# SpursLipu/YOLOv3v4-ModelCompression-MultidatasetTraining-Multibackbone

Hardware: AMD Instinct MI355X
Metric: images/sec YOLOv3-608 train fp16 (higher is better)
Workload: dtype f16; 1 GPU; YOLOv3 Darknet-53 608 COCO (80 classes) fp16 training step, batch 64/GPU: train-mode forward (batch-stat BN) + compute_loss + backward + nesterov SGD, single GPU; global_batch=64, parallelism=dp1

## Files before the change

yolov3v4-modelcompression-multidatasettraining-multibackbone_amd/csrc/conv_halo_pp.hip:

```cpp
#include "conv_igemm.h"

namespace yh {

template <typename T> struct HppMma;
template <> struct HppMma<f16> {
    typedef f16x8 frag_t;
    static __device__ __forceinline__ f32x4 mma(const frag_t& a, const frag_t& b, const f32x4& c) {
        return __builtin_amdgcn_mfma_f32_16x16x32_f16(a, b, c, 0, 0, 0);
    }
};
template <> struct HppMma<int8_t> {
    typedef i32x4 frag_t;
    static __device__ __forceinline__ i32x4 mma(const frag_t& a, const frag_t& b, const i32x4& c) {
        return __builtin_amdgcn_mfma_i32_16x16x64_i8(a, b, c, 0, 0, 0);
    }
};

template <typename T, int ACT, typename AccT>
__device__ __forceinline__ void hpp_epilogue(const ConvArgs& a, AccT (&acc)[8][4], const f32x4 (&bvs)[8], const long (&pix)[4],
                                             const int m0, const long tile_row, const int lane, float* const stage) {
    constexpr int TM = 8, TN = 4;
    const int mq = (lane >> 4) << 2, pc = lane & 15;
    T* const yg = reinterpret_cast<T*>(a.y);
    const T* const rg = reinterpret_cast<const T*>(a.res);
    const int mbase = m0 + mq;
    auto value = [&](auto ic, auto jc, int e) {
        constexpr int i = decltype(ic)::value, j = decltype(jc)::value;
        if constexpr (sizeof(T) == 1) {
            const float y = activate_q<ACT>((float)acc[i][j][e] * a.acc_scale + bvs[i][e], a.slope, a.inv_out_scale);
            return round_clamp_i8(y * a.inv_out_scale);
        } else {
            return activate_t<ACT, T>((float)acc[i][j][e] + bvs[i][e], a.slope);
        }
    };
    if constexpr (sizeof(T) != 1) {
        if (a.stats_part != nullptr) {
// ... 6 lines not shown
                    if (pix[j] >= 0) {
#pragma unroll
                        for (int e = 0; e < 4; ++e) {
                            const float q = (float)(T)value(ic, jc, e);
                            s1[e] += q;
                            s2[e] = fmaf(q, q, s2[e]);
                        }
                    }
                });
#pragma unroll
                for (int e = 0; e < 4; ++e) {
                    const float t1 = row16_sum(s1[e]), t2 = row16_sum(s2[e]);
                    const int m = mbase + i * 16 + e;
                    if (pc == 15 && stage != nullptr) {
                        stage[i * 16 + mq + e] = t1;
                        stage[128 + i * 16 + mq + e] = t2;
                    } else if (pc == 15 && m < a.Cout) {
                        row[m] = t1;
                        row[a.Cout + m] = t2;
                    }
                }
            });
            __builtin_amdgcn_wave_barrier();
            if (stage != nullptr) {
                const int half = lane >> 5, c4 = (lane & 31) * 4;
                const f32x4 sv = *reinterpret_cast<const f32x4*>(stage + half * 128 + c4);
                if (m0 + c4 < a.Cout) *reinterpret_cast<f32x4*>(row + half * a.Cout + m0 + c4) = sv;
            }
        }
    }
    const int k4 = lane >> 4;
    const int chan = ((k4 & 1) << 4) + ((k4 >> 1) << 3);
    const bool have_res = rg != nullptr;
    static_for<TN>([&](auto jc) {
        constexpr int j = decltype(jc)::value;
        const long p = pix[j];
        typedef unsigned int u32x2 __attribute__((ext_vector_type(2)));
        typedef typename std::conditional<sizeof(T) == 2, u32x4, u32x2>::type res8_t;
        res8_t rv[TM / 2];
        if (have_res) {
#pragma unroll
            for (int i2 = 0; i2 < TM / 2; ++i2) {
// ... 51 lines not shown
                }
                u32x2 o;
#pragma unroll
                for (int h = 0; h < 2; ++h)
                    o[h] = ((unsigned)(int)v[4 * h] & 0xffu) | (((unsigned)(int)v[4 * h + 1] & 0xffu) << 8) |
                           (((unsigned)(int)v[4 * h + 2] & 0xffu) << 16) | (((unsigned)(int)v[4 * h + 3] & 0xffu) << 24);
                *reinterpret_cast<u32x2*>(prow + m) = o;
            }
        });
    });
}

template <int T9, int LB> struct HppAllow {
    static constexpr int in(int t) { return (t >= 0 && t < LB) ? 1 : 0; }
    static constexpr int value = T9 == 8 ? 2 : 2 + in(T9 - 2) + in(T9 - 1) + in(T9);
};

template <int T9, int LB> struct HppAllow2 {
    static constexpr int in(int t) { return (t >= 0 && t < LB) ? 1 : 0; }
    static constexpr int end = T9 >= 7 ? 1 : 1 + in(T9 - 1) + in(T9);
    static constexpr int mid = T9 >= 7 ? 1 : 1 + in(T9 - 1);
};

struct HppDiv { unsigned m_img, s_img, m_wp, s_wp; };
__device__ __forceinline__ int hpp_div(int n, unsigned m, unsigned s) { return (int)(__umulhi((unsigned)n, m) >> s); }

template <typename T, int LB, int ROLE, int KFORM>
__global__ __launch_bounds__(512, 2) void conv3x3_hpp_kernel(const ConvArgs a, const int rows_hp, const int hbufs_arg, const HppDiv dv) {
    const int hbufs = hbufs_arg & 0xff;
    constexpr bool ONEBAR = KFORM == 1, REFRESH = KFORM == 2;
    constexpr int VEC = Prec<T>::VEC, BK = VEC * 4;
    constexpr int BM = 128, BN = 512, TM = 8, TN = 4, NW = 8, SA = 4;
    constexpr int A_CELLS = BM * 4;
    constexpr int LBR = ROLE ? 1 : LB;
    static_assert(sizeof(T) <= 2, "f16 / int8");
    typedef typename HppMma<T>::frag_t frag_t;
    typedef typename AccOf<T>::type acc_t;
    typedef const void __attribute__((address_space(1))) * gptr_t;
    typedef void __attribute__((address_space(3))) * lptr_t;

    extern __shared__ __attribute__((aligned(16))) u32x4 hsm[];
    u32x4* const Aring = hsm;
    u32x4* const Hbuf = hsm + SA * A_CELLS;
    u32x4* const dummy = Hbuf + hbufs * rows_hp * 4;
    int* const htab = reinterpret_cast<int*>(dummy + 64);

    const int lane = threadIdx.x & 63;
    const int wave = __builtin_amdgcn_readfirstlane(threadIdx.x >> 6);
    const int group = wave >> 2;

// ... 6 lines not shown
    {
        const int nb = gridDim.x, bid = blockIdx.x;
        const int q = nb >> 3, rr = nb & 7, xcd = bid & 7;
        const int logical = (xcd < rr ? xcd * (q + 1) : rr * (q + 1) + (xcd - rr) * q) + (bid >> 3);
        p_tile = logical / a.m_tiles;
        m_tile = logical - p_tile * a.m_tiles;
    }
    const int m0 = m_tile * BM;
    const long q0 = (long)p_tile * BN;
    const int Wp = a.W + 1;
    const int IMG = (a.H + 1) * Wp;

    const int lrow = lane >> 2;
    const int lu = (lane & 3) ^ (((lane >> 4) & 1) << 1);
    const T* const xg = reinterpret_cast<const T*>(a.x);
    const int wrow = (ROLE ? 2 * (wave & 3) : wave) * 16 + lrow;
    const T* const wsrc = reinterpret_cast<const T*>(a.w) + (long)min(m0 + wrow, a.m_pad - 1) * a.ktot + lu * VEC;
    const int wsrc2 = (min(m0 + wrow + 16, a.m_pad - 1) - min(m0 + wrow, a.m_pad - 1)) * a.ktot;
    auto halo_offset = [&](int j) {
        const int v = (int)q0 - Wp - 1 + j;
        int off = -1;
        if (j < rows_hp && v >= 0) {
            const int n = hpp_div(v, dv.m_img, dv.s_img);
            const int rem = v - n * IMG;
            const int yy = hpp_div(rem, dv.m_wp, dv.s_wp), xx = rem - yy * Wp;
            if (n < a.N && yy >= 1 && xx >= 1) off = ((n * a.H + yy - 1) * a.W + xx - 1) * a.ldx;
        }
        return off;
    };
    int boff[LBR];
    if constexpr (ROLE == 0) {
// ... 89 lines not shown
        LOADS;                                                \
        __builtin_amdgcn_sched_barrier(0);                    \
        asm volatile("s_waitcnt lgkmcnt(0)" ::: "memory");   \
        if (BAR_L) __builtin_amdgcn_s_barrier();              \
        __builtin_amdgcn_sched_barrier(0);                    \
        MMA;                                                  \
        __builtin_amdgcn_sched_barrier(0);                    \
        if (BAR_M) __builtin_amdgcn_s_barrier();              \
        __builtin_amdgcn_sched_barrier(0);                    \
    } while (0)

    const int nchunks = a.cin_k / BK;
    const int nk = 9 * nchunks;
    if constexpr (ROLE == 0) {
        static_for<LB>([&](auto ic) { issue_h(0, 0, ic); });
        issue_a(0, 0, 0);
        issue_a(1, 1, 0);
        issue_a(2, 2, 0);
        wait_vmcnt<2>();
    } else if (group == 0) {
        issue_a(0, 0, 0);
        issue_a(1, 1, 0);
        issue_a(2, 2, 0);
        wait_vmcnt<4>();
    } else {
        for (int i = 0; i < 6; ++i) issue_h2(0, 0, i);
        wait_vmcnt<0>();
    }
    if constexpr (REFRESH) {
        static_assert(!REFRESH || ROLE == 0, "the refresh form shares the LDS-DMA issue among all waves");
        wait_vmcnt<1>();
        YH_HPP_BARRIER();
        read_a(Aring, 0);
        read_b(Hbuf, 0);
// ... 47 lines not shown
                    fb[j] = *reinterpret_cast<frag_t*>(&v);
                    __builtin_amdgcn_sched_barrier(0);
                }
                if (group == 0) {
                    if (more_h) wait_vmcnt<HppAllow2<t, LB>::end>();
                    else if (s + 3 < nk) wait_vmcnt<1>();
                    else wait_vmcnt<0>();
                    YH_HPP_BARRIER();
                }
                ++s;
                st_r = (st_r + 1) & (SA - 1);
                st_w = (st_w + 1) & (SA - 1);
                if (++ptap == 9) { ptap = 0; pkc += BK; }
            });
        }
    } else {
    YH_HPP_BARRIER();
    if (!ONEBAR && group == 1) YH_HPP_BARRIER();
    int s = 0;
    int st_r = 0, st_w = 3;
    int ptap = 3, pkc = 0;
    for (int c = 0; c < nchunks; ++c) {
        const bool more_h = LB <= 7 ? c + 1 < nchunks : false;
        const u32x4* const hb = Hbuf + (c & (hbufs - 1)) * (rows_hp * 4);
        const int nbuf = (c + 1) & 1, nkc = (c + 1) * BK;
        static_for<9>([&](auto tc) {
            constexpr int t = decltype(tc)::value;
            const u32x4* const st = Aring + st_r * A_CELLS;
            const int tapoff = (t / 3) * Wp + (t % 3);
            constexpr int allow = HppAllow<t, LB>::value;
// ... 33 lines not shown
        const int m = m0 + i * 16 + mq;
        bvs[i] = m < a.Cout ? *reinterpret_cast<const f32x4*>(a.bias + m) : f32x4{0.f, 0.f, 0.f, 0.f};
    }
#pragma unroll
    for (int i = 0; i < TM; ++i) asm volatile("" ::"v"(bvs[i]));
    long pix[TN];
#pragma unroll
    for (int j = 0; j < TN; ++j) {
        const int q = (int)q0 + wave * 64 + j * 16 + r16;
        const int n = hpp_div(q, dv.m_img, dv.s_img);
        const int rem = q - n * IMG;
        const int yy = hpp_div(rem, dv.m_wp, dv.s_wp), xx = rem - yy * Wp;
        pix[j] = (n < a.N && yy >= 1 && xx >= 1) ? ((long)n * a.H + yy - 1) * a.W + xx - 1 : -1;
    }
    const long tile_row = (long)p_tile * NW + wave;
    float* const stage = (hbufs_arg >> 8) ? reinterpret_cast<float*>(reinterpret_cast<unsigned char*>(htab) + ((rows_hp * 4 + 15) & ~15)) + wave * 256 : nullptr;
    switch (a.act) {
        case YH_ACT_LEAKY: hpp_epilogue<T, YH_ACT_LEAKY>(a, acc, bvs, pix, m0, tile_row, lane, stage); break;
        case YH_ACT_MISH: hpp_epilogue<T, YH_ACT_MISH>(a, acc, bvs, pix, m0, tile_row, lane, stage); break;
        default: hpp_epilogue<T, YH_ACT_LINEAR>(a, acc, bvs, pix, m0, tile_row, lane, stage); break;
    }
}

#ifdef YH_HPP_PERSIST_AB
template <typename T, int LB>
__global__ __launch_bounds__(512, 2) void conv3x3_hpp_persist_kernel(const ConvArgs a, const int rows_hp, const HppDiv dv, const int total_tiles) {
    constexpr int VEC = Prec<T>::VEC, BK = VEC * 4;
    constexpr int BM = 128, BN = 512, TM = 8, TN = 4, NW = 8, SA = 4;
    constexpr int A_CELLS = BM * 4;
    static_assert(sizeof(T) <= 2, "f16 / int8");
    typedef typename HppMma<T>::frag_t frag_t;
    typedef typename AccOf<T>::type acc_t;
    typedef const void __attribute__((address_space(1))) * gptr_t;
    typedef void __attribute__((address_space(3))) * lptr_t;

// ... 184 lines not shown
            bvs[i] = m < ae.Cout ? *reinterpret_cast<const f32x4*>(ae.bias + m) : f32x4{0.f, 0.f, 0.f, 0.f};
        }
#pragma unroll
        for (int i = 0; i < TM; ++i) asm volatile("" ::"v"(bvs[i]));
        long pix[TN];
#pragma unroll
        for (int j = 0; j < TN; ++j) {
            const int q = q0 + wave * 64 + j * 16 + r16;
            const int n = hpp_div(q, dv.m_img, dv.s_img);
            const int rem = q - n * IMG;
            const int yy = hpp_div(rem, dv.m_wp, dv.s_wp), xx = rem - yy * Wp;
            pix[j] = (n < a.N && yy >= 1 && xx >= 1) ? ((long)n * a.H + yy - 1) * a.W + xx - 1 : -1;
        }
        const long tile_row = (long)p_tile * NW + wave;
        switch (ae.act) {
            case YH_ACT_LEAKY: hpp_epilogue<T, YH_ACT_LEAKY>(ae, acc, bvs, pix, m0, tile_row, lane, nullptr); break;
            case YH_ACT_MISH: hpp_epilogue<T, YH_ACT_MISH>(ae, acc, bvs, pix, m0, tile_row, lane, nullptr); break;
            default: hpp_epilogue<T, YH_ACT_LINEAR>(ae, acc, bvs, pix, m0, tile_row, lane, nullptr); break;
        }
        if (!has_next) break;
        vb = vnext;
        m_tile = m_next;
        p_tile = p_next;
        wsrc = weight_off(m_next * BM);
    }
#undef YH_HPP_PHASE
#undef YH_HPP_BARRIER
}

#endif

static void hpp_magic(unsigned d, unsigned* m, unsigned* s) {
    unsigned L = 0;
    while ((1ull << L) < d) ++L;
    const unsigned long long num = 1ull << (31 + L);
    *m = (unsigned)((num + d - 1) / d);
    *s = L - 1;
}

bool hpp_geometry(int W, int cin_k, int bk, int* rows_hp, int* lb, int* hbufs, size_t* lds) {
    const int Wp = W + 1;
    const int rows_h = 512 + 2 * Wp + 2;
    *rows_hp = ((rows_h + 15) / 16) * 16;
    const int groups = *rows_hp / 16;
    int l = (groups + 7) / 8;
    const int nchunks = cin_k / bk;
    *hbufs = nchunks > 1 ? 2 : 1;
    if (l == 8) l = 9;
    if (l < 5 || l > 9 || (nchunks > 1 && l > 7)) return false;
    *lb = l;
    *lds = ((size_t)4 * 128 * 4 + (size_t)*hbufs * *rows_hp * 4 + 64) * 16 + (size_t)*rows_hp * 4;
    return *lds <= 160 * 1024;
}

template <typename T, int LBV> static auto hpp_kern(int kform) -> void (*)(const ConvArgs, const int, const int, const HppDiv) {
#ifdef YH_HPP_ONEBAR_AB
    if constexpr (!(sizeof(T) == 1 && LBV == 7)) {
        if (kform == 1) return conv3x3_hpp_kernel<T, LBV, 0, 1>;
    }
#endif
#ifdef YH_HPP_REFRESH_AB
    if constexpr (LBV <= 7) {
        if (kform == 2) return conv3x3_hpp_kernel<T, LBV, 0, 2>;
    }
#endif
    (void)kform;
    return conv3x3_hpp_kernel<T, LBV, 0, 0>;
}

#ifndef YH_HPP_ONE_BARRIER_DEFAULT
#define YH_HPP_ONE_BARRIER_DEFAULT 0
#endif
#ifndef YH_HPP_KFORM_DEFAULT
#define YH_HPP_KFORM_DEFAULT 0
#endif
template <typename T> static int launch_hpp(const ConvArgs& a0, hipStream_t stream) {
    constexpr int BK = Prec<T>::VEC * 4;
    ConvArgs a = a0;
    if (a.R != 3 || a.S != 3 || a.stride != 1 || a.pad != 1 || a.ups != 1) return YH_EUNSUPPORTED;
    if (a.act != YH_ACT_LINEAR && a.act != YH_ACT_LEAKY && a.act != YH_ACT_MISH) return YH_EUNSUPPORTED;
    if (a.cin_k % BK) return YH_EALIGN;
    int rows_hp, lb, hbufs;
    size_t lds;
    if (!hpp_geometry(a.W, a.cin_k, BK, &rows_hp, &lb, &hbufs, &lds)) return YH_EUNSUPPORTED;
    if ((long)a.N * a.H * a.W * a.ldx + a.cin_k >= 0x7fffffffL || (long)a.m_pad * a.ktot >= 0x7fffffffL) return YH_EUNSUPPORTED;
    if ((long)(a.N + 1) * (a.H + 1) * (a.W + 1) + 4096 >= 0x7fffffffL) return YH_EUNSUPPORTED;
    const unsigned amask = sizeof(T) == 2 ? 15u : 7u;
    if (a.Cout % 8 || a.ldy % 8 || (((uintptr_t)a.y) & amask) || (a.res && (a.ldr % 8 || (((uintptr_t)a.res) & amask)))) return YH_EALIGN;
    a.m_tiles = (a.Cout + 127) / 128;
    const long Q = (long)a.N * (a.H + 1) * (a.W + 1);
    a.p_tiles = (int)((Q + 511) / 512);
    const long blocks = (long)a.m_tiles * a.p_tiles;
    if (blocks <= 0 || blocks > 0x7fffffffL) return YH_EINVAL;
    int stage_ok = 0;
    if (a.stats_part != nullptr && sizeof(T) == 2) {
        const char* e = getenv("YH_HPP_STATS_STAGE");
        const size_t base = (lds + 15) & ~(size_t)15;
        if (!(e && atoi(e) == 0) && base + 8192 <= 160 * 1024) {
            lds = base + 8192;
            stage_ok = 1;
        }
    }
    { const char* e = getenv("YH_HPP_STAGGER"); a.hpp_stagger = (e && blocks > 512) ? atoi(e) : 0; }
    HppDiv dv;
    hpp_magic((unsigned)((a.H + 1) * (a.W + 1)), &dv.m_img, &dv.s_img);
    hpp_magic((unsigned)(a.W + 1), &dv.m_wp, &dv.s_wp);
    const char* bar_env = getenv("YH_HPP_BARRIERS");
    const int one_bar = bar_env ? (atoi(bar_env) == 1 ? 1 : 0) : YH_HPP_ONE_BARRIER_DEFAULT;
    const char* form_env = getenv("YH_HPP_KFORM");
    const int kform = one_bar ? 1 : (form_env ? atoi(form_env) : YH_HPP_KFORM_DEFAULT);
#ifdef YH_HPP_ROLE_AB
    static const int role_env = [] { const char* e = getenv("YH_HPP_ROLE"); return e ? atoi(e) : 0; }();
    const int role = (role_env && rows_hp <= 768) ? 1 : 0;
#define YH_HPP_KERN(LBV) (role ? conv3x3_hpp_kernel<T, LBV, 1, 0> : hpp_kern<T, LBV>(kform))
#else
#define YH_HPP_KERN(LBV) hpp_kern<T, LBV>(kform)
#endif
#define YH_HPP_CASE(LBV)                                                                                                       \
    case LBV: {                                                                                                                \
        auto kern = YH_HPP_KERN(LBV);                                                                                          \
        hipError_t e = ensure_dynamic_lds(reinterpret_cast<const void*>(kern), lds);                         \
        if (e != hipSuccess) return (int)e;                                                                                    \
        hipLaunchKernelGGL(kern, dim3((unsigned)blocks), dim3(512), lds, stream, a, rows_hp, hbufs | (stage_ok << 8), dv);     \
        break;                                                                                                                 \
    }
    switch (lb) {
        YH_HPP_CASE(5) YH_HPP_CASE(6) YH_HPP_CASE(7) YH_HPP_CASE(9)
        default: return YH_EUNSUPPORTED;
    }
#undef YH_HPP_CASE
#undef YH_HPP_KERN
// ... 35 lines not shown
    switch (lb) {
        YH_HPPP_CASE(5) YH_HPPP_CASE(6) YH_HPPP_CASE(7)
        default: return YH_EUNSUPPORTED;
    }
#undef YH_HPPP_CASE
    return check_launch();
}

int launch_hpp_persist_tile(const ConvArgs& a, int dtype, hipStream_t stream) {
    if (dtype == YH_F16) return launch_hpp_persist<f16>(a, stream);
    if (dtype == YH_I8) return launch_hpp_persist<int8_t>(a, stream);
    return YH_EINVAL;
}
#endif

int launch_hpp_tile(const ConvArgs& a, int dtype, hipStream_t stream) {
#ifdef YH_HPP_PERSIST_AB
    static const bool persist = [] { const char* e = getenv("YH_HPP_PERSIST"); return e && atoi(e) != 0; }();
    if (persist && a.R == 3 && a.S == 3 && a.stride == 1 && a.pad == 1 && a.ups == 1) {
        const int bk = dtype == YH_I8 ? 64 : 32;
        const long tiles = (long)((a.Cout + 127) / 128) * (((long)a.N * (a.H + 1) * (a.W + 1) + 511) / 512);
        if (a.cin_k % bk == 0 && a.cin_k / bk >= 2 && tiles > 256) {
            const int rc = launch_hpp_persist_tile(a, dtype, stream);
            if (rc != YH_EUNSUPPORTED) return rc;
        }
    }
#endif
    if (dtype == YH_F16) return launch_hpp<f16>(a, stream);
    if (dtype == YH_I8) return launch_hpp<int8_t>(a, stream);
    return YH_EINVAL;
}

}
```

yolov3v4-modelcompression-multidatasettraining-multibackbone_amd/csrc/conv_igemm.h:

```cpp
#pragma once
#include <type_traits>

#include "common.h"

namespace yh {

struct ConvArgs {
    const void* x;
    const void* w;
    const float* bias;
    const void* res;
    void* y;
    int N, H, W, Cin, Ho, Wo, Cout, R, S, stride, pad;
    int ldx, ldr, ldy;
    int cin_k;
    int ktot;
    long P;
    int m_tiles, p_tiles;
    int m_pad;
    float acc_scale, out_scale, inv_out_scale;
    int act;
    float slope;
    int ups;
    float* stats_part;
// ... 448 lines not shown
                    store4<OutT>(dst + (long)(c.wo2 + 1) * a.ldy, v[0], v[1], v[2], v[3]);
                }
            }
        });
    });
}

int launch_k64_tile(const ConvArgs& a, int tile, int dtype, int out_f32, hipStream_t stream);
int launch_pointwise_tile(const ConvArgs& a, int dtype, int out_f32, hipStream_t stream);
int launch_stream3_tile(const ConvArgs& a, int dtype, hipStream_t stream);
long stream3_stats_rows(long P, int cout);
int launch_pwl_tile(const ConvArgs& a, int dtype, hipStream_t stream);
bool pwl_supported(int dtype, int out_f32, int cin, int cin_k, int cout, long P, int ldx, int ldy, int ldr, const void* x, const void* y,
                   const void* res, bool stats, bool bwd);
long pwl_stats_rows(long P, int cout, bool bwd = false);
int launch_hpp_tile(const ConvArgs& a, int dtype, hipStream_t stream);
bool hpp_geometry(int W, int cin_k, int bk, int* rows_hp, int* lb, int* hbufs, size_t* lds);

}
```

yolov3v4-modelcompression-multidatasettraining-multibackbone_amd/csrc/conv_igemm.hip:

```cpp
#include "conv_igemm.h"

namespace yh {

template <typename T, int TM, int TN, int KU> struct MmaStep;

template <int TM, int TN, int KU> struct MmaStep<f16, TM, TN, KU> {
    static __device__ __forceinline__ void run(const u32x4* As, const u32x4* Bs, int BM, int BN, int arow, int brow,
                                               int lane, f32x4 (&acc)[TM][TN]) {
        const int r = lane & 15;
#pragma unroll
        for (int h = 0; h < KU / 4; ++h) {
            const int u = h * 4 + (lane >> 4);
            f16x8 a[TM], b[TN];
#pragma unroll
            for (int i = 0; i < TM; ++i) {
                u32x4 v = As[u * BM + arow + i * 16 + r];
                a[i] = *reinterpret_cast<f16x8*>(&v);
            }
#pragma unroll
            for (int j = 0; j < TN; ++j) {
                u32x4 v = Bs[u * BN + brow + j * 16 + r];
                b[j] = *reinterpret_cast<f16x8*>(&v);
            }
#pragma unroll
// ... 727 lines not shown
        case 15: return launch<T, OutT, 128, 64, 2, 2, 8>(a, s);
        case 16: return launch<T, OutT, 256, 128, 4, 2, 8>(a, s);
        case 21: return launch_glds<T, OutT, 128, 128, 2, 2, 3>(a, s);
        case 22: return launch_glds<T, OutT, 64, 256, 1, 4, 3>(a, s);
        case 24: return launch_glds<T, OutT, 64, 128, 2, 2, 3>(a, s);
        case 25: return launch_glds<T, OutT, 128, 64, 2, 2, 3>(a, s);
        case 26: return launch_glds<T, OutT, 256, 128, 4, 2, 3>(a, s);
        case 27: return launch_glds<T, OutT, 128, 256, 2, 4, 3>(a, s);
        case 51: return launch_glds<T, OutT, 256, 128, 4, 2, 3, 1>(a, s);
        case 52: return launch_glds<T, OutT, 256, 128, 4, 2, 3, 2>(a, s);
        case 41: return launch_halo<T, OutT, 128>(a, s);
        case 42: return launch_halo<T, OutT, 256>(a, s);
        case 43:
            if constexpr (sizeof(T) == 2 && std::is_same<OutT, T>::value) return launch_hpp_tile(a, YH_F16, s);
            else return YH_EUNSUPPORTED;
        case 31: return launch_glds<T, OutT, 128, 128, 2, 2, 4>(a, s);
        case 61: case 62: case 63: case 64: case 65: case 66: case 67: case 68: case 69:
            if constexpr (sizeof(T) == 2) return launch_k64_tile(a, tile, YH_F16, std::is_same<OutT, float>::value ? 1 : 0, s);
            else return YH_EINVAL;
        case 32: return launch_glds<T, OutT, 64, 256, 1, 4, 4>(a, s);
        case 34: return launch_glds<T, OutT, 64, 128, 2, 2, 4>(a, s);
        case 35: return launch_glds<T, OutT, 128, 64, 2, 2, 4>(a, s);
        default: return YH_EINVAL;
    }
}

template <typename OutT> static int dispatch_tile_i8(const ConvArgs& a, int tile, hipStream_t s) {
    if (tile == 0) {
        tile = pick_tile(a.Cout, a.P, a.cin_k, 16);
        if (tile == 3) tile = 24;
    }
    switch (tile) {
        case 21: return launch_glds<int8_t, OutT, 128, 128, 2, 2, 3>(a, s);
        case 24: return launch_glds<int8_t, OutT, 64, 128, 2, 2, 3>(a, s);
        case 25: return launch_glds<int8_t, OutT, 128, 64, 2, 2, 3>(a, s);
        case 26: return launch_glds<int8_t, OutT, 256, 128, 4, 2, 3>(a, s);
        case 27: return launch_glds<int8_t, OutT, 128, 256, 2, 4, 3>(a, s);
        case 64: case 65: case 66: return launch_k64_tile(a, tile, YH_I8, std::is_same<OutT, float>::value ? 1 : 0, s);
        case 43:
            if constexpr (std::is_same<OutT, int8_t>::value) return launch_hpp_tile(a, YH_I8, s);
            else return YH_EUNSUPPORTED;
        default: return YH_EINVAL;
    }
}

__global__ void pack_qconv_weights_kernel(const float* __restrict__ qw, float inv_scale, const int32_t* __restrict__ cin_map,
                                          int cout, int cin, int taps, int cin_k, int8_t* __restrict__ packed) {
    const long total = (long)cout * cin * taps;
    for (long i = blockIdx.x * (long)blockDim.x + threadIdx.x; i < total; i += (long)gridDim.x * blockDim.x) {
        const int tap = (int)(i % taps);
        const long r = i / taps;
        const int ci = (int)(r % cin), co = (int)(r / cin);
        const int pc = cin_map ? cin_map[ci] : ci;
        packed[((long)co * taps + tap) * cin_k + pc] = (int8_t)(int)round_clamp_i8(qw[i] * inv_scale);
    }
}
// ... 31 lines not shown
        const long blocks = (long)((d->cout + bm - 1) / bm) * ((P + bn - 1) / bn);
        return (double)((blocks + 255) / 256) * (20000.0 + 3300.0 * nk);
    };
    const double c64 = pp(256, 256), c66 = d->cout >= 512 ? pp(512, 128) : 1e30;
    const double best = c64 < c66 ? c64 : c66;
    if (best > 0.95 * ring) return 0;
    return c66 <= c64 ? 66 : 64;
}

static bool pick_halo_tile(const yh_conv_desc* d) {
    if (d->dtype != YH_F16 || d->kh != 3 || d->kw != 3 || d->stride != 1 || d->pad != 1 || d->stats_ws || d->ups > 2) return false;
    if (d->cout != 128 && d->cout != 256) return false;
    return d->cin >= 128 && d->cin % 32 == 0 && d->w_in >= 48 && d->w_in <= 96 && (long)d->n * d->h * d->w_in >= 131072;
}

static bool pick_hpp_tile(const yh_conv_desc* d) {
    static const bool off = getenv("YH_NO_HPP") != nullptr;
    if (off || (d->dtype != YH_F16 && d->dtype != YH_I8) || d->out_f32) return false;
    if (d->kh != 3 || d->kw != 3 || d->stride != 1 || d->pad != 1 || d->ups != 1) return false;
    if (d->act != YH_ACT_LINEAR && d->act != YH_ACT_LEAKY && d->act != YH_ACT_MISH) return false;
    const int bk = d->dtype == YH_I8 ? 64 : 32;
    if (d->cin_k % bk || d->cout < 64 || d->cin_k / bk < 2) return false;
    if (d->dtype == YH_F16 && d->cout <= 64 && d->cin_k / bk == 2) return false;
    if (d->dtype == YH_I8 && d->cin_k / bk == 2 && (d->res || (long)d->n * d->ho * d->wo < 262144)) return false;
    const unsigned amask = d->dtype == YH_F16 ? 15u : 7u;
    if (d->cout % 8 || d->ldy % 8 || (((uintptr_t)d->y) & amask) || (d->res && (d->ldr % 8 || (((uintptr_t)d->res) & amask)))) return false;
    if ((long)(d->n + 1) * (d->h + 1) * (d->w_in + 1) + 4096 >= 0x7fffffffL) return false;
    int rows_hp, lb, hbufs;
    size_t lds;
    if (!yh::hpp_geometry(d->w_in, d->cin_k, bk, &rows_hp, &lb, &hbufs, &lds)) return false;
    if ((long)d->n * d->h * d->w_in * d->ldx + d->cin_k >= 0x7fffffffL || (long)d->m_pad * 9 * d->cin_k >= 0x7fffffffL) return false;
    const long blocks = (long)((d->cout + 127) / 128) * (((long)d->n * (d->h + 1) * (d->w_in + 1) + 511) / 512);
    const long rounds = (blocks + 255) / 256;
    return blocks >= 192 && (rounds >= 4 || blocks * 100 >= rounds * 256 * 60);
}

static bool pick_pointwise_tile(const yh_conv_desc* d) {
    static const bool off = getenv("YH_NO_POINTWISE") != nullptr;
    if (off || (d->dtype != YH_F16 && d->dtype != YH_I8)) return false;
    if (d->kh != 1 || d->kw != 1 || d->stride != 1 || d->pad != 0 || d->ups != 1 || d->res || d->stats_ws) return false;
    if (d->act != YH_ACT_LINEAR && d->act != YH_ACT_LEAKY && d->act != YH_ACT_MISH) return false;
    const int k = d->dtype == YH_I8 ? 64 : 32;
    if (d->cin != d->cin_k || d->cin_k % k || d->cout > 128) return false;
    const int mt = d->cout <= 32 ? 2 : (d->cout <= 64 ? 4 : 8), ks = d->cin_k / k;
    if (!((mt == 2 && (ks == 1 || ks == 2 || ks == 4)) || (mt == 4 && (ks == 1 || ks == 2)) || (mt == 8 && ks == 1))) return false;
    return (long)d->n * d->ho * d->wo >= 262144;
}

static bool stream3_supported(const yh_conv_desc* d) {
// ... 23 lines not shown
    return yh::pwl_supported(d->dtype, d->out_f32, d->cin, d->cin_k, d->cout, (long)d->n * d->ho * d->wo, d->ldx, d->ldy, d->ldr, d->x, d->y,
                             d->res, !bwd && d->stats_ws != nullptr, bwd);
}
static bool pick_pwl_tile(const yh_conv_desc* d) {
    static const bool off = getenv("YH_NO_PWL") != nullptr;
    static const long min_px = [] { const char* e = getenv("YH_PWL_MIN_PIXELS"); return e ? atol(e) : 262144L; }();
    return !off && pwl_desc_supported(d) && (long)d->n * d->ho * d->wo >= min_px;
}

extern "C" int yh_conv2d_tile(const yh_conv_desc* d) {
    if (!d) return YH_EINVAL;
    if (d->tile != 0) return d->tile;
    if (pick_pointwise_tile(d)) return 71;
    if (pick_pwl_tile(d)) return 73;
    if (pick_stream3_tile(d)) return 72;
    if (pick_hpp_tile(d)) return 43;
    if (pick_halo_tile(d)) return 41;
    if (const int pp = pick_pp_tile(d)) return pp;
    const int t = yh::pick_tile(d->cout, (long)d->n * d->ho * d->wo, d->cin_k, d->dtype == YH_F16 ? 8 : 4, d->kh * d->kw);
    if (d->ups == 2 && (t == 21 || t == 26 || t == 27 || t == 25)) {
        if (d->dtype == YH_F16) return 24;
        if (d->dtype == YH_I8) return 25;
    }
    if (d->dtype == YH_I8 && (t == 21 || t == 27) && (long)d->cin_k * d->kh * d->kw <= 256) return 25;
    return (d->dtype == YH_I8 && t == 3) ? 24 : t;
}

static bool tile_geometry(int tile, int* bn, int* wn) {
    switch (tile) {
        case 1: case 11: case 21: case 31: *bn = 128; *wn = 2; return true;
        case 2: case 12: case 22: case 32: case 3: *bn = 256; *wn = 4; return true;
// ... 12 lines not shown
    if (d->dtype != YH_F16 || d->bwd_ldz % 8 || !yh::aligned16(d->bwd_z) || (d->tile != 0 && d->tile != 73)) return 0;
    static const bool off = getenv("YH_NO_BWD_SUMS") != nullptr;
    if (off || !pick_pwl_tile(d)) return 0;
    return (int64_t)yh::pwl_stats_rows((long)d->n * d->ho * d->wo, d->cout, true);
}

extern "C" int64_t yh_conv2d_stats_rows(const yh_conv_desc* d) {
    if (!d || d->n <= 0 || d->ho <= 0 || d->wo <= 0 || d->dtype == YH_I8) return 0;
    if (d->bwd_z) return 0;
    int bn, wn;
    yh_conv_desc q = *d;
    if (!q.stats_ws) q.stats_ws = reinterpret_cast<float*>(sizeof(float));
    const int tile = yh_conv2d_tile(&q);
    if (tile == 72) return (int64_t)yh::stream3_stats_rows((long)d->n * d->ho * d->wo, d->cout);
    if (tile == 73) return (int64_t)yh::pwl_stats_rows((long)d->n * d->ho * d->wo, d->cout);
    if (tile == 43)
        return (int64_t)(((long)d->n * (d->h + 1) * (d->w_in + 1) + 511) / 512) * 8;
    if (!tile_geometry(tile, &bn, &wn)) return 0;
    const long P = (long)d->n * d->ho * d->wo;
    return (int64_t)((P + bn - 1) / bn) * wn;
}

static void qadd_pow2_args(yh::ConvArgs& a) {
    const char* env = getenv("YH_QADD_POW2");
    if (env && env[0] == '0') return;
    int e[5];
    const float f[5] = {a.q_rx, a.q_ra, a.q_scale_x, a.q_scale_a, a.q_inv_scale_sum};
    for (int i = 0; i < 5; ++i) {
        int ex;
        if (!(f[i] > 0.f) || frexpf(f[i], &ex) != 0.5f) return;
        e[i] = ex - 1;
// ... 56 lines not shown
    a.stats_part = nullptr;
    a.bz = nullptr;
    a.bgamma = a.bbeta = a.bmean = a.binvstd = nullptr;
    a.ldbz = a.bact = 0;
    a.bslope = 0.f;
    if (d->bwd_z) {
        const int64_t rows = yh_conv2d_bwd_stats_rows(d);
        if (rows <= 0) return YH_EUNSUPPORTED;
        if (!d->stats_ws || d->stats_ws_floats < rows * 2 * d->cout) return YH_EINVAL;
        a.stats_part = d->stats_ws;
        a.bz = d->bwd_z; a.ldbz = d->bwd_ldz; a.bact = d->bwd_act; a.bslope = d->bwd_slope;
        a.bgamma = d->bwd_gamma; a.bbeta = d->bwd_beta; a.bmean = d->bwd_mean; a.binvstd = d->bwd_invstd;
        return launch_pwl_tile(a, d->dtype, (hipStream_t)stream);
    }
    if (d->stats_ws) {
        if (d->ups != 1 || d->res || d->dtype == YH_I8 || (d->tile >= 40 && d->tile < 50 && d->tile != 43)) return YH_EINVAL;
        const int64_t rows = yh_conv2d_stats_rows(d);
        if (rows <= 0 || d->stats_ws_floats < rows * 2 * d->cout) return YH_EINVAL;
        a.stats_part = d->stats_ws;
    }
    hipStream_t s = (hipStream_t)stream;
    int tile = d->tile;
    if (tile == 0) {
        tile = yh_conv2d_tile(d);
        if (d->ups == 4 && !(tile >= 21 && tile <= 35)) tile = 24;
    }
    if (tile == 71) {
        if (d->kh != 1 || d->kw != 1 || d->stride != 1 || d->pad != 0 || d->ups != 1 || d->res || d->stats_ws || d->cin != d->cin_k ||
            d->cout > 128 || d->dtype == YH_F32) return YH_EUNSUPPORTED;
        return launch_pointwise_tile(a, d->dtype, d->out_f32, s);
    }
// ... 17 lines not shown
```

Measured before the change: 1232 images/s.

## Add 64-row output-channel variant of halo 3x3 conv kernel with cost-model selection

```diff
diff --git a/yolov3v4-modelcompression-multidatasettraining-multibackbone_amd/csrc/conv_halo_pp.hip b/yolov3v4-modelcompression-multidatasettraining-multibackbone_amd/csrc/conv_halo_pp.hip
--- a/yolov3v4-modelcompression-multidatasettraining-multibackbone_amd/csrc/conv_halo_pp.hip
+++ b/yolov3v4-modelcompression-multidatasettraining-multibackbone_amd/csrc/conv_halo_pp.hip
@@ -16,10 +16,10 @@
     }
 };
 
-template <typename T, int ACT, typename AccT>
-__device__ __forceinline__ void hpp_epilogue(const ConvArgs& a, AccT (&acc)[8][4], const f32x4 (&bvs)[8], const long (&pix)[4],
+template <typename T, int ACT, int TM, typename AccT>
+__device__ __forceinline__ void hpp_epilogue(const ConvArgs& a, AccT (&acc)[TM][4], const f32x4 (&bvs)[TM], const long (&pix)[4],
                                              const int m0, const long tile_row, const int lane, float* const stage) {
-    constexpr int TM = 8, TN = 4;
+    constexpr int TN = 4, BMW = TM * 16;
     const int mq = (lane >> 4) << 2, pc = lane & 15;
     T* const yg = reinterpret_cast<T*>(a.y);
     const T* const rg = reinterpret_cast<const T*>(a.res);
@@ -56,7 +56,7 @@
                     const int m = mbase + i * 16 + e;
                     if (pc == 15 && stage != nullptr) {
                         stage[i * 16 + mq + e] = t1;
-                        stage[128 + i * 16 + mq + e] = t2;
+                        stage[BMW + i * 16 + mq + e] = t2;
                     } else if (pc == 15 && m < a.Cout) {
                         row[m] = t1;
                         row[a.Cout + m] = t2;
@@ -66,8 +66,10 @@
             __builtin_amdgcn_wave_barrier();
             if (stage != nullptr) {
                 const int half = lane >> 5, c4 = (lane & 31) * 4;
-                const f32x4 sv = *reinterpret_cast<const f32x4*>(stage + half * 128 + c4);
-                if (m0 + c4 < a.Cout) *reinterpret_cast<f32x4*>(row + half * a.Cout + m0 + c4) = sv;
+                if (c4 < BMW) {
+                    const f32x4 sv = *reinterpret_cast<const f32x4*>(stage + half * BMW + c4);
+                    if (m0 + c4 < a.Cout) *reinterpret_cast<f32x4*>(row + half * a.Cout + m0 + c4) = sv;
+                }
             }
         }
     }
@@ -149,6 +151,7 @@
 template <int T9, int LB> struct HppAllow {
     static constexpr int in(int t) { return (t >= 0 && t < LB) ? 1 : 0; }
     static constexpr int value = T9 == 8 ? 2 : 2 + in(T9 - 2) + in(T9 - 1) + in(T9);
+    static constexpr int halo_only = value - 2;
 };
 
 template <int T9, int LB> struct HppAllow2 {
@@ -160,15 +163,17 @@
 struct HppDiv { unsigned m_img, s_img, m_wp, s_wp; };
 __device__ __forceinline__ int hpp_div(int n, unsigned m, unsigned s) { return (int)(__umulhi((unsigned)n, m) >> s); }
 
-template <typename T, int LB, int ROLE, int KFORM>
+template <typename T, int LB, int ROLE, int KFORM, int MH = 8>
 __global__ __launch_bounds__(512, 2) void conv3x3_hpp_kernel(const ConvArgs a, const int rows_hp, const int hbufs_arg, const HppDiv dv) {
     const int hbufs = hbufs_arg & 0xff;
     constexpr bool ONEBAR = KFORM == 1, REFRESH = KFORM == 2;
     constexpr int VEC = Prec<T>::VEC, BK = VEC * 4;
-    constexpr int BM = 128, BN = 512, TM = 8, TN = 4, NW = 8, SA = 4;
+    constexpr int BM = MH * 16, BN = 512, TM = MH, TN = 4, NW = 8, SA = 4;
     constexpr int A_CELLS = BM * 4;
+    constexpr bool HALF = MH == 4;
     constexpr int LBR = ROLE ? 1 : LB;
     static_assert(sizeof(T) <= 2, "f16 / int8");
+    static_assert(MH == 8 || (MH == 4 && ROLE == 0 && KFORM == 0), "the 64-row tile exists for the shipped schedule only");
     typedef typename HppMma<T>::frag_t frag_t;
     typedef typename AccOf<T>::type acc_t;
     typedef const void __attribute__((address_space(1))) * gptr_t;
@@ -205,7 +210,8 @@
     const int lrow = lane >> 2;
     const int lu = (lane & 3) ^ (((lane >> 4) & 1) << 1);
     const T* const xg = reinterpret_cast<const T*>(a.x);
-    const int wrow = (ROLE ? 2 * (wave & 3) : wave) * 16 + lrow;
+    const int wrow = (ROLE ? 2 * (wave & 3) : (HALF ? wave & 3 : wave)) * 16 + lrow;
+    const bool wpiece = !HALF || wave < 4;
     const T* const wsrc = reinterpret_cast<const T*>(a.w) + (long)min(m0 + wrow, a.m_pad - 1) * a.ktot + lu * VEC;
     const int wsrc2 = (min(m0 + wrow + 16, a.m_pad - 1) - min(m0 + wrow, a.m_pad - 1)) * a.ktot;
     auto halo_offset = [&](int j) {
@@ -325,10 +331,14 @@
     const int nk = 9 * nchunks;
     if constexpr (ROLE == 0) {
         static_for<LB>([&](auto ic) { issue_h(0, 0, ic); });
-        issue_a(0, 0, 0);
-        issue_a(1, 1, 0);
-        issue_a(2, 2, 0);
-        wait_vmcnt<2>();
+        if (wpiece) {
+            issue_a(0, 0, 0);
+            issue_a(1, 1, 0);
+            issue_a(2, 2, 0);
+            wait_vmcnt<2>();
+        } else {
+            wait_vmcnt<0>();
+        }
     } else if (group == 0) {
         issue_a(0, 0, 0);
         issue_a(1, 1, 0);
@@ -406,6 +416,44 @@
                 if (++ptap == 9) { ptap = 0; pkc += BK; }
             });
         }
+    } else if constexpr (HALF) {
+    YH_HPP_BARRIER();
+    if (group == 1) YH_HPP_BARRIER();
+    int s = 0;
+    int st_r = 0, st_w = 3;
+    int ptap = 3, pkc = 0;
+    for (int c = 0; c < nchunks; ++c) {
+        const bool more_h = LB <= 7 ? c + 1 < nchunks : false;
+        const u32x4* const hb = Hbuf + (c & (hbufs - 1)) * (rows_hp * 4);
+        const int nbuf = (c + 1) & 1, nkc = (c + 1) * BK;
+        static_for<9>([&](auto tc) {
+            constexpr int t = decltype(tc)::value;
+            const u32x4* const st = Aring + st_r * A_CELLS;
+            const int tapoff = (t / 3) * Wp + (t % 3);
+            constexpr int allow = HppAllow<t, LB>::value;
+            constexpr int allow_h = HppAllow<t, LB>::halo_only;
+            YH_HPP_PHASE({
+                read_a(st, 0);
+                read_b(hb, tapoff);
+                if (wpiece && s + 3 < nk) issue_a(st_w, ptap, pkc);
+                if constexpr (t < LB) { if (more_h) issue_h(nbuf, nkc, tc); }
+                if (wpiece) {
+                    if (more_h) wait_vmcnt<allow>();
+                    else {
+                        const int rem = nk - 2 - s;
+                        if (rem >= 2) wait_vmcnt<2>(); else if (rem == 1) wait_vmcnt<1>(); else wait_vmcnt<0>();
+                    }
+                } else {
+                    if (more_h) wait_vmcnt<allow_h>(); else wait_vmcnt<0>();
+                }
+            }, mma(H0{}), true, true);
+            ++s;
+            st_r = (st_r + 1) & (SA - 1);
+            st_w = (st_w + 1) & (SA - 1);
+            if (++ptap == 9) { ptap = 0; pkc += BK; }
+        });
+    }
+    if (group == 0) YH_HPP_BARRIER();
     } else {
     YH_HPP_BARRIER();
     if (!ONEBAR && group == 1) YH_HPP_BARRIER();
@@ -469,11 +517,11 @@
         pix[j] = (n < a.N && yy >= 1 && xx >= 1) ? ((long)n * a.H + yy - 1) * a.W + xx - 1 : -1;
     }
     const long tile_row = (long)p_tile * NW + wave;
-    float* const stage = (hbufs_arg >> 8) ? reinterpret_cast<float*>(reinterpret_cast<unsigned char*>(htab) + ((rows_hp * 4 + 15) & ~15)) + wave * 256 : nullptr;
+    float* const stage = (hbufs_arg >> 8) ? reinterpret_cast<float*>(reinterpret_cast<unsigned char*>(htab) + ((rows_hp * 4 + 15) & ~15)) + wave * (2 * BM) : nullptr;
     switch (a.act) {
-        case YH_ACT_LEAKY: hpp_epilogue<T, YH_ACT_LEAKY>(a, acc, bvs, pix, m0, tile_row, lane, stage); break;
-        case YH_ACT_MISH: hpp_epilogue<T, YH_ACT_MISH>(a, acc, bvs, pix, m0, tile_row, lane, stage); break;
-        default: hpp_epilogue<T, YH_ACT_LINEAR>(a, acc, bvs, pix, m0, tile_row, lane, stage); break;
+        case YH_ACT_LEAKY: hpp_epilogue<T, YH_ACT_LEAKY, TM>(a, acc, bvs, pix, m0, tile_row, lane, stage); break;
+        case YH_ACT_MISH: hpp_epilogue<T, YH_ACT_MISH, TM>(a, acc, bvs, pix, m0, tile_row, lane, stage); break;
+        default: hpp_epilogue<T, YH_ACT_LINEAR, TM>(a, acc, bvs, pix, m0, tile_row, lane, stage); break;
     }
 }
 
@@ -688,9 +736,9 @@
         }
         const long tile_row = (long)p_tile * NW + wave;
         switch (ae.act) {
-            case YH_ACT_LEAKY: hpp_epilogue<T, YH_ACT_LEAKY>(ae, acc, bvs, pix, m0, tile_row, lane, nullptr); break;
-            case YH_ACT_MISH: hpp_epilogue<T, YH_ACT_MISH>(ae, acc, bvs, pix, m0, tile_row, lane, nullptr); break;
-            default: hpp_epilogue<T, YH_ACT_LINEAR>(ae, acc, bvs, pix, m0, tile_row, lane, nullptr); break;
+            case YH_ACT_LEAKY: hpp_epilogue<T, YH_ACT_LEAKY, TM>(ae, acc, bvs, pix, m0, tile_row, lane, nullptr); break;
+            case YH_ACT_MISH: hpp_epilogue<T, YH_ACT_MISH, TM>(ae, acc, bvs, pix, m0, tile_row, lane, nullptr); break;
+            default: hpp_epilogue<T, YH_ACT_LINEAR, TM>(ae, acc, bvs, pix, m0, tile_row, lane, nullptr); break;
         }
         if (!has_next) break;
         vb = vnext;
@@ -712,7 +760,7 @@
     *s = L - 1;
 }
 
-bool hpp_geometry(int W, int cin_k, int bk, int* rows_hp, int* lb, int* hbufs, size_t* lds) {
+bool hpp_geometry(int W, int cin_k, int bk, int* rows_hp, int* lb, int* hbufs, size_t* lds, int ring_rows) {
     const int Wp = W + 1;
     const int rows_h = 512 + 2 * Wp + 2;
     *rows_hp = ((rows_h + 15) / 16) * 16;
@@ -723,11 +771,16 @@
     if (l == 8) l = 9;
     if (l < 5 || l > 9 || (nchunks > 1 && l > 7)) return false;
     *lb = l;
-    *lds = ((size_t)4 * 128 * 4 + (size_t)*hbufs * *rows_hp * 4 + 64) * 16 + (size_t)*rows_hp * 4;
+    *lds = ((size_t)4 * ring_rows * 4 + (size_t)*hbufs * *rows_hp * 4 + 64) * 16 + (size_t)*rows_hp * 4;
     return *lds <= 160 * 1024;
 }
 
-template <typename T, int LBV> static auto hpp_kern(int kform) -> void (*)(const ConvArgs, const int, const int, const HppDiv) {
+template <typename T, int LBV, int MH> static auto hpp_kern(int kform) -> void (*)(const ConvArgs, const int, const int, const HppDiv) {
+    if constexpr (MH == 4) {
+        (void)kform;
+        if constexpr (LBV == 9) return nullptr;
+        else return conv3x3_hpp_kernel<T, LBV, 0, 0, 4>;
+    } else {
 #ifdef YH_HPP_ONEBAR_AB
     if constexpr (!(sizeof(T) == 1 && LBV == 7)) {
         if (kform == 1) return conv3x3_hpp_kernel<T, LBV, 0, 1>;
@@ -740,6 +793,7 @@
 #endif
     (void)kform;
     return conv3x3_hpp_kernel<T, LBV, 0, 0>;
+    }
 }
 
 #ifndef YH_HPP_ONE_BARRIER_DEFAULT
@@ -748,20 +802,21 @@
 #ifndef YH_HPP_KFORM_DEFAULT
 #define YH_HPP_KFORM_DEFAULT 0
 #endif
-template <typename T> static int launch_hpp(const ConvArgs& a0, hipStream_t stream) {
-    constexpr int BK = Prec<T>::VEC * 4;
+template <typename T, int MH> static int launch_hpp(const ConvArgs& a0, hipStream_t stream) {
+    constexpr int BK = Prec<T>::VEC * 4, BM = MH * 16;
     ConvArgs a = a0;
     if (a.R != 3 || a.S != 3 || a.stride != 1 || a.pad != 1 || a.ups != 1) return YH_EUNSUPPORTED;
     if (a.act != YH_ACT_LINEAR && a.act != YH_ACT_LEAKY && a.act != YH_ACT_MISH) return YH_EUNSUPPORTED;
     if (a.cin_k % BK) return YH_EALIGN;
     int rows_hp, lb, hbufs;
     size_t lds;
-    if (!hpp_geometry(a.W, a.cin_k, BK, &rows_hp, &lb, &hbufs, &lds)) return YH_EUNSUPPORTED;
+    if (!hpp_geometry(a.W, a.cin_k, BK, &rows_hp, &lb, &hbufs, &lds, BM)) return YH_EUNSUPPORTED;
+    if (MH == 4 && lb == 9) return YH_EUNSUPPORTED;
     if ((long)a.N * a.H * a.W * a.ldx + a.cin_k >= 0x7fffffffL || (long)a.m_pad * a.ktot >= 0x7fffffffL) return YH_EUNSUPPORTED;
     if ((long)(a.N + 1) * (a.H + 1) * (a.W + 1) + 4096 >= 0x7fffffffL) return YH_EUNSUPPORTED;
     const unsigned amask = sizeof(T) == 2 ? 15u : 7u;
     if (a.Cout % 8 || a.ldy % 8 || (((uintptr_t)a.y) & amask) || (a.res && (a.ldr % 8 || (((uintptr_t)a.res) & amask)))) return YH_EALIGN;
-    a.m_tiles = (a.Cout + 127) / 128;
+    a.m_tiles = (a.Cout + BM - 1) / BM;
     const long Q = (long)a.N * (a.H + 1) * (a.W + 1);
     a.p_tiles = (int)((Q + 511) / 512);
     const long blocks = (long)a.m_tiles * a.p_tiles;
@@ -769,9 +824,9 @@
     int stage_ok = 0;
     if (a.stats_part != nullptr && sizeof(T) == 2) {
         const char* e = getenv("YH_HPP_STATS_STAGE");
-        const size_t base = (lds + 15) & ~(size_t)15;
-        if (!(e && atoi(e) == 0) && base + 8192 <= 160 * 1024) {
-            lds = base + 8192;
+        const size_t base = (lds + 15) & ~(size_t)15, rows_bytes = (size_t)8 * 2 * BM * sizeof(float);
+        if (!(e && atoi(e) == 0) && base + rows_bytes <= 160 * 1024) {
+            lds = base + rows_bytes;
             stage_ok = 1;
         }
     }
@@ -785,10 +840,10 @@
     const int kform = one_bar ? 1 : (form_env ? atoi(form_env) : YH_HPP_KFORM_DEFAULT);
 #ifdef YH_HPP_ROLE_AB
     static const int role_env = [] { const char* e = getenv("YH_HPP_ROLE"); return e ? atoi(e) : 0; }();
-    const int role = (role_env && rows_hp <= 768) ? 1 : 0;
-#define YH_HPP_KERN(LBV) (role ? conv3x3_hpp_kernel<T, LBV, 1, 0> : hpp_kern<T, LBV>(kform))
+    const int role = (role_env && rows_hp <= 768 && MH == 8) ? 1 : 0;
+#define YH_HPP_KERN(LBV) (role ? conv3x3_hpp_kernel<T, LBV, 1, 0> : hpp_kern<T, LBV, MH>(kform))
 #else
-#define YH_HPP_KERN(LBV) hpp_kern<T, LBV>(kform)
+#define YH_HPP_KERN(LBV) hpp_kern<T, LBV, MH>(kform)
 #endif
 #define YH_HPP_CASE(LBV)                                                                                                       \
     case LBV: {                                                                                                                \
@@ -854,10 +909,10 @@
 }
 #endif
 
-int launch_hpp_tile(const ConvArgs& a, int dtype, hipStream_t stream) {
+int launch_hpp_tile(const ConvArgs& a, int dtype, hipStream_t stream, bool half_rows) {
 #ifdef YH_HPP_PERSIST_AB
     static const bool persist = [] { const char* e = getenv("YH_HPP_PERSIST"); return e && atoi(e) != 0; }();
-    if (persist && a.R == 3 && a.S == 3 && a.stride == 1 && a.pad == 1 && a.ups == 1) {
+    if (persist && !half_rows && a.R == 3 && a.S == 3 && a.stride == 1 && a.pad == 1 && a.ups == 1) {
         const int bk = dtype == YH_I8 ? 64 : 32;
         const long tiles = (long)((a.Cout + 127) / 128) * (((long)a.N * (a.H + 1) * (a.W + 1) + 511) / 512);
         if (a.cin_k % bk == 0 && a.cin_k / bk >= 2 && tiles > 256) {
@@ -866,8 +921,12 @@
         }
     }
 #endif
-    if (dtype == YH_F16) return launch_hpp<f16>(a, stream);
-    if (dtype == YH_I8) return launch_hpp<int8_t>(a, stream);
+    if (half_rows) {
+        if (dtype == YH_F16) return launch_hpp<f16, 4>(a, stream);
+        return dtype == YH_I8 ? YH_EUNSUPPORTED : YH_EINVAL;
+    }
+    if (dtype == YH_F16) return launch_hpp<f16, 8>(a, stream);
+    if (dtype == YH_I8) return launch_hpp<int8_t, 8>(a, stream);
     return YH_EINVAL;
 }
 
diff --git a/yolov3v4-modelcompression-multidatasettraining-multibackbone_amd/csrc/conv_igemm.h b/yolov3v4-modelcompression-multidatasettraining-multibackbone_amd/csrc/conv_igemm.h
--- a/yolov3v4-modelcompression-multidatasettraining-multibackbone_amd/csrc/conv_igemm.h
+++ b/yolov3v4-modelcompression-multidatasettraining-multibackbone_amd/csrc/conv_igemm.h
@@ -486,7 +486,7 @@
 bool pwl_supported(int dtype, int out_f32, int cin, int cin_k, int cout, long P, int ldx, int ldy, int ldr, const void* x, const void* y,
                    const void* res, bool stats, bool bwd);
 long pwl_stats_rows(long P, int cout, bool bwd = false);
-int launch_hpp_tile(const ConvArgs& a, int dtype, hipStream_t stream);
-bool hpp_geometry(int W, int cin_k, int bk, int* rows_hp, int* lb, int* hbufs, size_t* lds);
-
-}
+int launch_hpp_tile(const ConvArgs& a, int dtype, hipStream_t stream, bool half_rows = false);
+bool hpp_geometry(int W, int cin_k, int bk, int* rows_hp, int* lb, int* hbufs, size_t* lds, int ring_rows = 128);
+
+}
diff --git a/yolov3v4-modelcompression-multidatasettraining-multibackbone_amd/csrc/conv_igemm.hip b/yolov3v4-modelcompression-multidatasettraining-multibackbone_amd/csrc/conv_igemm.hip
--- a/yolov3v4-modelcompression-multidatasettraining-multibackbone_amd/csrc/conv_igemm.hip
+++ b/yolov3v4-modelcompression-multidatasettraining-multibackbone_amd/csrc/conv_igemm.hip
@@ -765,6 +765,9 @@
         case 43:
             if constexpr (sizeof(T) == 2 && std::is_same<OutT, T>::value) return launch_hpp_tile(a, YH_F16, s);
             else return YH_EUNSUPPORTED;
+        case 44:
+            if constexpr (sizeof(T) == 2 && std::is_same<OutT, T>::value) return launch_hpp_tile(a, YH_F16, s, true);
+            else return YH_EUNSUPPORTED;
         case 31: return launch_glds<T, OutT, 128, 128, 2, 2, 4>(a, s);
         case 61: case 62: case 63: case 64: case 65: case 66: case 67: case 68: case 69:
             if constexpr (sizeof(T) == 2) return launch_k64_tile(a, tile, YH_F16, std::is_same<OutT, float>::value ? 1 : 0, s);
@@ -791,6 +794,7 @@
         case 43:
             if constexpr (std::is_same<OutT, int8_t>::value) return launch_hpp_tile(a, YH_I8, s);
             else return YH_EUNSUPPORTED;
+        case 44: return YH_EUNSUPPORTED;
         default: return YH_EINVAL;
     }
 }
@@ -852,25 +856,42 @@
     return d->cin >= 128 && d->cin % 32 == 0 && d->w_in >= 48 && d->w_in <= 96 && (long)d->n * d->h * d->w_in >= 131072;
 }
 
-static bool pick_hpp_tile(const yh_conv_desc* d) {
+static int pick_hpp_tile(const yh_conv_desc* d) {
     static const bool off = getenv("YH_NO_HPP") != nullptr;
-    if (off || (d->dtype != YH_F16 && d->dtype != YH_I8) || d->out_f32) return false;
-    if (d->kh != 3 || d->kw != 3 || d->stride != 1 || d->pad != 1 || d->ups != 1) return false;
-    if (d->act != YH_ACT_LINEAR && d->act != YH_ACT_LEAKY && d->act != YH_ACT_MISH) return false;
+    if (off || (d->dtype != YH_F16 && d->dtype != YH_I8) || d->out_f32) return 0;
+    if (d->kh != 3 || d->kw != 3 || d->stride != 1 || d->pad != 1 || d->ups != 1) return 0;
+    if (d->act != YH_ACT_LINEAR && d->act != YH_ACT_LEAKY && d->act != YH_ACT_MISH) return 0;
     const int bk = d->dtype == YH_I8 ? 64 : 32;
-    if (d->cin_k % bk || d->cout < 64 || d->cin_k / bk < 2) return false;
-    if (d->dtype == YH_F16 && d->cout <= 64 && d->cin_k / bk == 2) return false;
-    if (d->dtype == YH_I8 && d->cin_k / bk == 2 && (d->res || (long)d->n * d->ho * d->wo < 262144)) return false;
+    if (d->cin_k % bk || d->cout < 64 || d->cin_k / bk < 2) return 0;
     const unsigned amask = d->dtype == YH_F16 ? 15u : 7u;
-    if (d->cout % 8 || d->ldy % 8 || (((uintptr_t)d->y) & amask) || (d->res && (d->ldr % 8 || (((uintptr_t)d->res) & amask)))) return false;
-    if ((long)(d->n + 1) * (d->h + 1) * (d->w_in + 1) + 4096 >= 0x7fffffffL) return false;
+    if (d->cout % 8 || d->ldy % 8 || (((uintptr_t)d->y) & amask) || (d->res && (d->ldr % 8 || (((uintptr_t)d->res) & amask)))) return 0;
+    if ((long)(d->n + 1) * (d->h + 1) * (d->w_in + 1) + 4096 >= 0x7fffffffL) return 0;
+    if ((long)d->n * d->h * d->w_in * d->ldx + d->cin_k >= 0x7fffffffL || (long)d->m_pad * 9 * d->cin_k >= 0x7fffffffL) return 0;
+    const long p_tiles = ((long)d->n * (d->h + 1) * (d->w_in + 1) + 511) / 512;
+    const long nk = 9L * (d->cin_k / bk);
+    auto fills = [](long blocks) {
+        const long rounds = (blocks + 255) / 256;
+        return blocks >= 192 && (rounds >= 4 || blocks * 100 >= rounds * 256 * 60);
+    };
     int rows_hp, lb, hbufs;
     size_t lds;
-    if (!yh::hpp_geometry(d->w_in, d->cin_k, bk, &rows_hp, &lb, &hbufs, &lds)) return false;
-    if ((long)d->n * d->h * d->w_in * d->ldx + d->cin_k >= 0x7fffffffL || (long)d->m_pad * 9 * d->cin_k >= 0x7fffffffL) return false;
-    const long blocks = (long)((d->cout + 127) / 128) * (((long)d->n * (d->h + 1) * (d->w_in + 1) + 511) / 512);
-    const long rounds = (blocks + 255) / 256;
-    return blocks >= 192 && (rounds >= 4 || blocks * 100 >= rounds * 256 * 60);
+    const long blocks43 = (long)((d->cout + 127) / 128) * p_tiles, blocks44 = (long)((d->cout + 63) / 64) * p_tiles;
+    bool ok43 = yh::hpp_geometry(d->w_in, d->cin_k, bk, &rows_hp, &lb, &hbufs, &lds) && fills(blocks43);
+    const bool thin2 = d->dtype == YH_F16 && d->cout <= 64 && d->cin_k / bk == 2;
+    if (thin2) ok43 = false;
+    if (d->dtype == YH_I8 && d->cin_k / bk == 2 && (d->res || (long)d->n * d->ho * d->wo < 262144)) ok43 = false;
+    const char* half_env = getenv("YH_HPP_HALF");
+    const int half_mode = half_env ? (atoi(half_env) != 0 ? 1 : 0) : -1;
+    const bool ok44 = half_mode != 0 && d->dtype == YH_F16 && yh::hpp_geometry(d->w_in, d->cin_k, bk, &rows_hp, &lb, &hbufs, &lds, 64) &&
+                      lb != 9 && fills(blocks44);
+    if (ok44 && half_mode == 1) return 44;
+    if (ok44 && ok43) {
+        const double c43 = (double)((blocks43 + 255) / 256) * (29000.0 + 1024.0 * nk);
+        const double c44 = (double)((blocks44 + 255) / 256) * (17000.0 + 760.0 * nk);
+        if (c44 < 0.9 * c43) return 44;
+    }
+    if (ok44 && thin2 && !d->stats_ws && (long)d->n * d->ho * d->wo >= (1L << 20)) return 44;
+    return ok43 ? 43 : 0;
 }
 
 static bool pick_pointwise_tile(const yh_conv_desc* d) {
@@ -924,7 +945,7 @@
     if (pick_pointwise_tile(d)) return 71;
     if (pick_pwl_tile(d)) return 73;
     if (pick_stream3_tile(d)) return 72;
-    if (pick_hpp_tile(d)) return 43;
+    if (const int hpp = pick_hpp_tile(d)) return hpp;
     if (pick_halo_tile(d)) return 41;
     if (const int pp = pick_pp_tile(d)) return pp;
     const int t = yh::pick_tile(d->cout, (long)d->n * d->ho * d->wo, d->cin_k, d->dtype == YH_F16 ? 8 : 4, d->kh * d->kw);
@@ -967,7 +988,7 @@
     const int tile = yh_conv2d_tile(&q);
     if (tile == 72) return (int64_t)yh::stream3_stats_rows((long)d->n * d->ho * d->wo, d->cout);
     if (tile == 73) return (int64_t)yh::pwl_stats_rows((long)d->n * d->ho * d->wo, d->cout);
-    if (tile == 43)
+    if (tile == 43 || tile == 44)
         return (int64_t)(((long)d->n * (d->h + 1) * (d->w_in + 1) + 511) / 512) * 8;
     if (!tile_geometry(tile, &bn, &wn)) return 0;
     const long P = (long)d->n * d->ho * d->wo;
@@ -1054,7 +1075,7 @@
         return launch_pwl_tile(a, d->dtype, (hipStream_t)stream);
     }
     if (d->stats_ws) {
-        if (d->ups != 1 || d->res || d->dtype == YH_I8 || (d->tile >= 40 && d->tile < 50 && d->tile != 43)) return YH_EINVAL;
+        if (d->ups != 1 || d->res || d->dtype == YH_I8 || (d->tile >= 40 && d->tile < 50 && d->tile != 43 && d->tile != 44)) return YH_EINVAL;
         const int64_t rows = yh_conv2d_stats_rows(d);
         if (rows <= 0 || d->stats_ws_floats < rows * 2 * d->cout) return YH_EINVAL;
         a.stats_part = d->stats_ws;
```

Result: no change. 1231 images/s (-0.0%).
